# evroon/mav-detection

Hardware: AMD Instinct MI355X
Metric: frame-pairs/sec at 1920x1080 (higher is better)
Workload: dtype f32; 1 GPU; 1920x1080, batch 64 per GPU, Farneback + FoE + phi/threshold + box; global_batch=64, parallelism=frame-parallel x1, record_exchange=none (1 GPU), torch_in_process=False

## Files before the change

mav-detection_amd/csrc/kernels_flow.hip:

```cpp
#include "mavflow_internal.h"

#include <algorithm>
#include <type_traits>

static __device__ __forceinline__ int clampi(int v, int lo, int hi) { return v < lo ? lo : (v > hi ? hi : v); }

struct TileMap { int tiles_x, tiles_y, per_img, n_tiles, strip_w, xcd, ty0; };
static __device__ __forceinline__ bool tile_of_block(const TileMap& tm, int* s, int* tx, int* ty)
{
    const int per = ((int)gridDim.x + 7) >> 3;
    const int tile = tm.xcd ? (int)(blockIdx.x & 7) * per + (int)(blockIdx.x >> 3) : (int)blockIdx.x;
    if (tile >= tm.n_tiles) return false;
    const int img = tile / tm.per_img;
    int tr = tile - img * tm.per_img;
    const int strip_tiles = tm.strip_w * tm.tiles_y;
    const int st = tr / strip_tiles;
    tr -= st * strip_tiles;
    const int x_base = st * tm.strip_w;
    const int sw = min(tm.strip_w, tm.tiles_x - x_base);
    const int row = tr / sw;
    *s = img; *ty = row + tm.ty0; *tx = x_base + tr - row * sw;
    return true;
}
static TileMap make_tile_map(int w, int h, int G, int tile_w, int tile_h, int ty0 = 0, int ty1 = -1, int strip = 0)
// ... 625 lines not shown
    return p;
}
bool blur_resize_is_fused(int W, int H, int w, int h, int ksize, int esize)
{
    if (!(!(w == W && h == H) && ksize <= 13 && H > 2 * ksize && W > 2 * ksize && (size_t)fused_blur_rows(H, h, ksize) * 256 <= 48 * 1024))
        return false;
    if (esize == 1) return true;
    const int pitch = staged_pitch_words(W, w, ksize);
    return fused_lds_bytes(fused_blur_rows(H, h, ksize), pitch, esize) <= 64 * 1024;
}

template <typename T>
static __device__ __forceinline__ void blur3_block(const T* __restrict__ src, float* __restrict__ dst, int W, int H, int bx, int by)
{
    typedef typename QuadOf<T>::type Q;
    const int x = (bx * 64 + (threadIdx.x & 63)) * 4;
    const int y0 = (by * 4 + (threadIdx.x >> 6)) * 4;
    if (x >= W || y0 >= H) return;
    const int xl = x == 0 ? 1 : x - 1;
    const int xr = x + 4 >= W ? W - 2 : x + 4;
    Q qs[6];
    T ls[6], rs[6];
#pragma unroll
    for (int r = 0; r < 6; r++) {
        int yy = y0 - 1 + r;
        yy = yy < 0 ? -yy : (yy >= H ? 2 * H - 2 - yy : yy);
        yy = yy < 0 ? 0 : (yy >= H ? H - 1 : yy);
        const T* p = src + (size_t)yy * W;
        qs[r] = *(const Q*)(p + x);
        ls[r] = p[xl];
        rs[r] = p[xr];
    }
    float hrow[6][4];
#pragma unroll
    for (int r = 0; r < 6; r++) {
        if constexpr (sizeof(T) == 1) {
            const uint32_t q = qs[r];
            const float a = (float)ls[r], b0 = (float)(q & 255u), b1 = (float)((q >> 8) & 255u), b2 = (float)((q >> 16) & 255u),
                        b3 = (float)(q >> 24), c = (float)rs[r];
            hrow[r][0] = 0.5f * b0 + 0.25f * (a + b1);
            hrow[r][1] = 0.5f * b1 + 0.25f * (b0 + b2);
            hrow[r][2] = 0.5f * b2 + 0.25f * (b1 + b3);
            hrow[r][3] = 0.5f * b3 + 0.25f * (b2 + c);
        } else {
            float b[4];
            quad_px<T>(qs[r], b);
            const float a = (float)ls[r], c = (float)rs[r];
            hrow[r][0] = 0.5f * b[0] + 0.25f * (a + b[1]);
            hrow[r][1] = 0.5f * b[1] + 0.25f * (b[0] + b[2]);
            hrow[r][2] = 0.5f * b[2] + 0.25f * (b[1] + b[3]);
            hrow[r][3] = 0.5f * b[3] + 0.25f * (b[2] + c);
        }
    }
#pragma unroll
    for (int r = 0; r < 4; r++) {
        float4 o;
        o.x = 0.5f * hrow[r + 1][0] + 0.25f * (hrow[r][0] + hrow[r + 2][0]);
        o.y = 0.5f * hrow[r + 1][1] + 0.25f * (hrow[r][1] + hrow[r + 2][1]);
        o.z = 0.5f * hrow[r + 1][2] + 0.25f * (hrow[r][2] + hrow[r + 2][2]);
        o.w = 0.5f * hrow[r + 1][3] + 0.25f * (hrow[r][3] + hrow[r + 2][3]);
        if (y0 + r < H) *(float4*)(dst + (size_t)(y0 + r) * W + x) = o;
    }
}

template <typename T, int PATH>
__global__ __launch_bounds__(256) void k_blur_multi(const T* __restrict__ img, const T* __restrict__ img2, int split, size_t img_stride,
                                                    int W, int H, int dword_ok, BlurJobs jobs)
{
    extern __shared__ __attribute__((aligned(16))) float hrows[];
    int k = 0;
    for (int i = 1; i < jobs.n; i++) k = (int)blockIdx.x >= jobs.j[i].first_block ? i : k;
    const BlurJob J = jobs.j[k];
    const int b = (int)blockIdx.x - J.first_block;
    const int z = b / (J.gx * J.gy), rem = b - z * J.gx * J.gy;
    const int by = rem / J.gx, bx = rem - by * J.gx;
    const T* base = image_of(img, img2, split, img_stride, z);
    float* out = J.out + (size_t)z * J.out_stride;
    if (J.fused) blur_fused_any<T, PATH>(base, out, W, H, J.w, J.h, J.bp, J.rows_cap, J.pitch_w, dword_ok, J.th, bx, by, hrows);
    else blur3_block(base, out, W, H, bx, by);
}
template <typename T>
static int quad_ok(const FrameRun<T>& f)
{
    const uintptr_t m = 4 * sizeof(T) - 1;
    return (f.W % 4 == 0 && f.img_stride % 4 == 0 && ((uintptr_t)f.img & m) == 0 && ((uintptr_t)f.img2 & m) == 0) ? 1 : 0;
}
template <typename T>
static bool blur3_fast_ok(const FrameRun<T>& f, const LayerTarget& t)
{
    return t.w == f.W && t.h == f.H && t.bp.fixed3 && f.W >= 8 && f.H >= 2 && quad_ok(f) && t.out_stride % 4 == 0 &&
           ((uintptr_t)t.out & 15) == 0;
}
template <typename T>
bool blur_multi_ok(const FrameRun<T>& f, const LayerTarget& t)
{
    return blur3_fast_ok(f.runs(), t) || blur_resize_is_fused(f.W, f.H, t.w, t.h, t.bp.ksize, (int)sizeof(T));
}
template <typename T>
static void blur_multi_launch(hipStream_t st, const FrameRun<T>& f, int dword_ok, BlurJobs jobs)
{
    const int esize = (int)sizeof(T), W = f.W, H = f.H;
    int blocks = 0;
    size_t lds = 0;
    for (int i = 0; i < jobs.n; i++) {
        BlurJob& J = jobs.j[i];
        J.fused = !(J.w == W && J.h == H);
        if (J.fused) {
            const FusedPlan fp = fused_plan(W, H, J.w, J.h, J.bp, dword_ok, esize);
            J.rows_cap = fp.rows; J.pitch_w = fp.pitch_w; J.th = fp.th;
            J.gx = (J.w + 63) / 64; J.gy = (J.h + fp.th - 1) / fp.th;
            lds = std::max(lds, fp.lds);
        } else {
            J.rows_cap = J.pitch_w = 0;
            J.gx = (W / 4 + 63) / 64; J.gy = ((H + 3) / 4 + 3) / 4;
        }
        J.first_block = blocks;
        blocks += J.gx * J.gy * f.G;
    }
    int path = -1;
    for (int i = 0; i < jobs.n; i++)
        if (jobs.j[i].fused) {
            const int p = fused_path_of(jobs.j[i].bp, jobs.j[i].pitch_w, dword_ok, esize);
            path = path < 0 ? p : (path == p ? p : FP_ANY);
        }
    with_fused_path<T>(path, [&](auto P) {
        hipLaunchKernelGGL((k_blur_multi<T, decltype(P)::value>), dim3(blocks), dim3(256), lds, st, f.img, f.img2, f.split, f.img_stride, W, H,
                           dword_ok, jobs);
    });
}
template <typename T>
void launch_blur_multi(hipStream_t st, const FrameRun<T>& frames, BlurJobs jobs)
{
    const FrameRun<T> f = frames.runs();
    const int dword_ok = quad_ok(f);
    const int esize = (int)sizeof(T);
    if (f.G <= 8) return blur_multi_launch(st, f, dword_ok, jobs);
    bool done[MAV_MAX_JOBS] = {false};
    for (int i = 0; i < jobs.n; i++) {
        if (done[i]) continue;
        auto path_of = [&](const BlurJob& J) {
            if (J.w == f.W && J.h == f.H) return -1;
            const FusedPlan fp = fused_plan(f.W, f.H, J.w, J.h, J.bp, dword_ok, esize);
            return fused_path_of(J.bp, fp.pitch_w, dword_ok, esize);
        };
        const int p = path_of(jobs.j[i]);
        BlurJobs sub{0, 0, {}};
        for (int k = i; k < jobs.n; k++)
            if (!done[k] && path_of(jobs.j[k]) == p) { sub.j[sub.n++] = jobs.j[k]; done[k] = true; }
        blur_multi_launch(st, f, dword_ok, sub);
    }
}

template <typename T>
__global__ __launch_bounds__(256) void k_blur3(const T* __restrict__ img, const T* __restrict__ img2, int split,
                                               size_t img_stride, int W, int H, float* __restrict__ out, size_t out_stride)
{
    blur3_block(image_of(img, img2, split, img_stride, blockIdx.z), out + (size_t)blockIdx.z * out_stride, W, H, blockIdx.x, blockIdx.y);
}

template <typename T>
bool blur_resize_needs_tmp(const FrameRun<T>& f, const LayerTarget& t)
{
    return !blur3_fast_ok(f.runs(), t) && !blur_resize_is_fused(f.W, f.H, t.w, t.h, t.bp.ksize, (int)sizeof(T));
}
template <typename T>
void launch_blur_resize(hipStream_t st, const FrameRun<T>& frames, const LayerTarget& t, const BlurScratch& scratch)
{
    const FrameRun<T> f = frames.runs();
    const int G = f.G, W = f.W, H = f.H, w = t.w, h = t.h;
    const BlurParams& bp = t.bp;
    if (blur3_fast_ok(f, t)) {
        dim3 grid((W / 4 + 63) / 64, ((H + 3) / 4 + 3) / 4, G);
        hipLaunchKernelGGL(k_blur3<T>, grid, dim3(256), 0, st, f.img, f.img2, f.split, f.img_stride, W, H, t.out, t.out_stride);
        return;
    }
    const int dword_ok = quad_ok(f);
    const int esize = (int)sizeof(T);
    const int pitch_w = staged_pitch_words(W, w, bp.ksize);
    if (!scratch.two_pass && blur_resize_is_fused(W, H, w, h, bp.ksize, esize)) {
        const FusedPlan fp = fused_plan(W, H, w, h, bp, dword_ok, esize);
        const dim3 grid((w + 63) / 64, (h + fp.th - 1) / fp.th, G);
        with_fused_path<T>(fused_path_of(bp, fp.pitch_w, dword_ok, esize), [&](auto P) {
            if constexpr (decltype(P)::value != FP_ANY)
                hipLaunchKernelGGL((k_blur_resize_fused<T, decltype(P)::value>), grid, dim3(256), fp.lds, st, f.img, f.img2, f.split, f.img_stride,
                                   W, H, w, h, bp, t.out, t.out_stride, fp.rows, fp.pitch_w, dword_ok, fp.th);
        });
        return;
    }
    int rows_blk = 16;
    while (rows_blk > 4 && (size_t)rows_blk * pitch_w * 4 * esize > 48 * 1024) rows_blk >>= 1;
    if ((size_t)rows_blk * pitch_w * 4 * esize <= 48 * 1024)
    {
        const int gx = (w + 63) / 64, nby = (H + rows_blk - 1) / rows_blk;
        const int gy = nby;
        const size_t lds_h = (size_t)((rows_blk * pitch_w * esize + 1) & ~1) * 4 + (size_t)((bp.ksize + 4) & ~3) * 8;
        hipLaunchKernelGGL(k_blur_resize_h<T>, dim3(gx, gy, G), dim3(256), lds_h, st, f.img, f.img2, f.split, f.img_stride, W, H, w, bp,
                           scratch.tmp, scratch.stride, rows_blk, pitch_w, dword_ok);
    }
    else
        hipLaunchKernelGGL(k_blur_resize_h_direct<T>, dim3((w + 63) / 64, ((H + 3) / 4 + 3) / 4, G), dim3(256), 0, st, f.img, f.img2, f.split,
                           f.img_stride, W, H, w, bp, scratch.tmp, scratch.stride);
    hipLaunchKernelGGL(k_blur_resize_v, dim3((w + 63) / 64, (h + 3) / 4, G), dim3(256), 0, st, (const float*)scratch.tmp, scratch.stride, H, w,
                       h, bp, t.out, t.out_stride);
}
#define MAV_BLUR_DEPTH(T)                                                                                     \
    template bool blur_multi_ok<T>(const FrameRun<T>&, const LayerTarget&);                                   \
    template void launch_blur_multi<T>(hipStream_t, const FrameRun<T>&, BlurJobs);                            \
    template bool blur_resize_needs_tmp<T>(const FrameRun<T>&, const LayerTarget&);                           \
    template void launch_blur_resize<T>(hipStream_t, const FrameRun<T>&, const LayerTarget&, const BlurScratch&);
MAV_BLUR_DEPTH(uint8_t)
MAV_BLUR_DEPTH(uint16_t)
MAV_BLUR_DEPTH(float)
#undef MAV_BLUR_DEPTH

#define PX 64
#define PY 16
struct __attribute__((packed, aligned(4))) F2U { float x, y; };
struct __attribute__((packed, aligned(4))) F4U { float x, y, z, w; };
static __device__ __forceinline__ void load5(const float* __restrict__ p, float v[5])
{
    const F4U a = *(const F4U*)p;
    v[0] = a.x; v[1] = a.y; v[2] = a.z; v[3] = a.w; v[4] = p[4];
}
static __device__ __forceinline__ void store5(float* __restrict__ p, const float v[5])
{
    *(F4U*)p = F4U{v[0], v[1], v[2], v[3]};
    p[4] = v[4];
}
template <int N_T>
static __device__ __forceinline__ void polyexp_tile(const float* __restrict__ src, float* __restrict__ dst, int w, int h, const PolyCoef& pc,
                                                    int tile_x, int tile_y, float* __restrict__ smem)
{
    const int n = N_T > 0 ? N_T : pc.n;
    const int EX = PX + 2 * n, EY = PY + 2 * n;
    float* tile = smem;
    float* v0 = tile + EX * EY;
    float* v1 = v0 + PY * EX;
    float* v2 = v1 + PY * EX;
    const int tid = threadIdx.x;
    const int x0 = tile_x * PX, y0 = tile_y * PY;

    if constexpr (N_T > 0) {
        constexpr int TOT = (PX + 2 * N_T) * (PY + 2 * N_T), CNT = (TOT + 255) / 256;
        float v[CNT];
#pragma unroll
        for (int j = 0; j < CNT; j++) {
            const int i = tid + 256 * j;
            if (i < TOT) {
                const int ly = i / EX, lx = i - ly * EX;
                const int gx = clampi(x0 - n + lx, 0, w - 1), gy = clampi(y0 - n + ly, 0, h - 1);
                v[j] = src[(size_t)gy * w + gx];
            }
        }
#pragma unroll
        for (int j = 0; j < CNT; j++)
            if (tid + 256 * j < TOT) tile[tid + 256 * j] = v[j];
    } else {
        for (int i = tid; i < EX * EY; i += 256) {
            const int ly = i / EX, lx = i - ly * EX;
            const int gx = clampi(x0 - n + lx, 0, w - 1), gy = clampi(y0 - n + ly, 0, h - 1);
            tile[i] = src[(size_t)gy * w + gx];
        }
    }
    __syncthreads();
    for (int i = tid; i < PY * EX; i += 256) {
        const int ly = i / EX, lx = i - ly * EX;
        const float* c = tile + (ly + n) * EX + lx;
        float t0 = c[0] * pc.g[0], t1 = 0.f, t2 = 0.f;
#pragma unroll
        for (int k = 1; k <= n; k++) {
            const float a = c[-k * EX], b = c[k * EX];
            const float p = a + b;
            t0 = fmaf(pc.g[k], p, t0);
            t1 = fmaf(pc.xg[k], b - a, t1);
            t2 = fmaf(pc.xxg[k], p, t2);
        }
        v0[i] = t0; v1[i] = t1; v2[i] = t2;
    }
    __syncthreads();
    for (int i = tid; i < PY * PX; i += 256) {
        const int ly = i >> 6, lx = i & 63;
        const int gx = x0 + lx, gy = y0 + ly;
        if (gx >= w || gy >= h) continue;
        const float* p0 = v0 + ly * EX + lx + n;
        const float* p1 = v1 + ly * EX + lx + n;
        const float* p2 = v2 + ly * EX + lx + n;
        float b1 = p0[0] * pc.g[0], b2 = 0.f, b3 = p1[0] * pc.g[0], b4 = 0.f, b5 = p2[0] * pc.g[0], b6 = 0.f;
#pragma unroll
        for (int k = 1; k <= n; k++) {
            const float a0 = p0[-k], c0 = p0[k], a1 = p1[-k], c1 = p1[k], a2 = p2[-k], c2 = p2[k];
            const float tg = c0 + a0;
            b1 = fmaf(tg, pc.g[k], b1);
            b4 = fmaf(tg, pc.xxg[k], b4);
            b2 = fmaf(c0 - a0, pc.xg[k], b2);
            b3 = fmaf(c1 + a1, pc.g[k], b3);
            b6 = fmaf(c1 - a1, pc.xg[k], b6);
            b5 = fmaf(c2 + a2, pc.g[k], b5);
        }
        const float r[5] = {b3 * pc.ig11, b2 * pc.ig11, fmaf(b5, pc.ig33, b1 * pc.ig03), fmaf(b4, pc.ig33, b1 * pc.ig03), b6 * pc.ig55};
        store5(dst + 5 * ((size_t)gy * w + gx), r);
    }
}

template <int N_T>
__global__ __launch_bounds__(256) void k_polyexp(const float* __restrict__ I, size_t I_stride, int w, int h, PolyCoef pc, TileMap tm,
                                                 float* __restrict__ R, size_t R_stride)
{
    int img_s, tile_x, tile_y;
    if (!tile_of_block(tm, &img_s, &tile_x, &tile_y)) return;
    extern __shared__ __attribute__((aligned(16))) float smem[];
    polyexp_tile<N_T>(I + (size_t)img_s * I_stride, R + (size_t)img_s * R_stride, w, h, pc, tile_x, tile_y, smem);
}

template <int N_T>
__global__ __launch_bounds__(256) void k_polyexp_multi(PolyJobs jobs, PolyCoef pc)
{
    int k = 0;
    for (int i = 1; i < jobs.n; i++) k = (int)blockIdx.x >= jobs.j[i].first_block ? i : k;
    const PolyJob J = jobs.j[k];
    const int tile = (int)blockIdx.x - J.first_block;
    const int img_s = tile / J.per_img, rem = tile - img_s * J.per_img;
    const int tile_y = rem / J.tiles_x, tile_x = rem - tile_y * J.tiles_x;
    extern __shared__ __attribute__((aligned(16))) float smem[];
    polyexp_tile<N_T>(J.I + (size_t)img_s * J.I_stride, J.R + (size_t)img_s * J.R_stride, J.w, J.h, pc, tile_x, tile_y, smem);
}
void launch_polyexp_multi(hipStream_t st, PolyJobs jobs, int G, const PolyCoef& pc)
{
    const int n = pc.n;
    const size_t lds = sizeof(float) * ((size_t)(PX + 2 * n) * (PY + 2 * n) + 3 * (size_t)PY * (PX + 2 * n));
    int blocks = 0;
    for (int i = 0; i < jobs.n; i++) {
        PolyJob& J = jobs.j[i];
        J.tiles_x = (J.w + PX - 1) / PX;
        J.per_img = J.tiles_x * ((J.h + PY - 1) / PY);
        J.first_block = blocks;
        blocks += J.per_img * G;
    }
    if (n == 8) hipLaunchKernelGGL(k_polyexp_multi<8>, dim3(blocks), dim3(256), lds, st, jobs, pc);
    else if (n == 7) hipLaunchKernelGGL(k_polyexp_multi<7>, dim3(blocks), dim3(256), lds, st, jobs, pc);
    else if (n == 5) hipLaunchKernelGGL(k_polyexp_multi<5>, dim3(blocks), dim3(256), lds, st, jobs, pc);
    else hipLaunchKernelGGL(k_polyexp_multi<0>, dim3(blocks), dim3(256), lds, st, jobs, pc);
}

void launch_polyexp(hipStream_t st, const float* I, size_t I_stride, int G, int w, int h, const PolyCoef& pc, float* R,
                    size_t R_stride)
{
    const int n = pc.n;
    const size_t lds = sizeof(float) * ((size_t)(PX + 2 * n) * (PY + 2 * n) + 3 * (size_t)PY * (PX + 2 * n));
    TileMap tm = make_tile_map(w, h, G, PX, PY);
    tm.xcd = 0;
    const dim3 grid(tile_grid(tm));
    if (n == 8)
        hipLaunchKernelGGL(k_polyexp<8>, grid, dim3(256), lds, st, I, I_stride, w, h, pc, tm, R, R_stride);
    else if (n == 7)
        hipLaunchKernelGGL(k_polyexp<7>, grid, dim3(256), lds, st, I, I_stride, w, h, pc, tm, R, R_stride);
    else if (n == 5)
        hipLaunchKernelGGL(k_polyexp<5>, grid, dim3(256), lds, st, I, I_stride, w, h, pc, tm, R, R_stride);
    else
        hipLaunchKernelGGL(k_polyexp<0>, grid, dim3(256), lds, st, I, I_stride, w, h, pc, tm, R, R_stride);
}

struct GatherPx {
    float p00[5], p01[5], p10[5], p11[5];
    float fx, fy;
    bool inside;
};
static __device__ __forceinline__ void gather_row(const float* __restrict__ p, float a[5], float b[5])
{
    const F4U t0 = *(const F4U*)p, t1 = *(const F4U*)(p + 4);
    const F2U t2 = *(const F2U*)(p + 8);
    a[0] = t0.x; a[1] = t0.y; a[2] = t0.z; a[3] = t0.w; a[4] = t1.x;
    b[0] = t1.y; b[1] = t1.z; b[2] = t1.w; b[3] = t2.x; b[4] = t2.y;
}
static __device__ __forceinline__ void gather_issue(const float* __restrict__ R1p, int w, int h, int x, int y, float dx, float dy, GatherPx& g)
{
    float fx = x + dx, fy = y + dy;
    const int x1 = (int)floorf(fx), y1 = (int)floorf(fy);
    g.fx = fx - x1; g.fy = fy - y1;
    g.inside = (unsigned)x1 < (unsigned)(w - 1) && (unsigned)y1 < (unsigned)(h - 1);
    const int xc = g.inside ? x1 : 0, yc = g.inside ? y1 : 0;
    const float* p = R1p + 5 * ((size_t)yc * w + xc);
    const size_t row = (w > 1 && h > 1) ? 5 * (size_t)w : 0;
    gather_row(p, g.p00, g.p01);
    gather_row(p + row, g.p10, g.p11);
}
static __device__ __forceinline__ void gather_inside(const float* __restrict__ R1p, int w, int h, int x, int y, float dx, float dy, GatherPx& g)
{
    float fx = x + dx, fy = y + dy;
    const int x1 = (int)floorf(fx), y1 = (int)floorf(fy);
    g.fx = fx - x1; g.fy = fy - y1;
    g.inside = (unsigned)x1 < (unsigned)(w - 1) && (unsigned)y1 < (unsigned)(h - 1);
    if (!g.inside) return;
    const float* p = R1p + 5 * ((size_t)y1 * w + x1);
    gather_row(p, g.p00, g.p01);
    gather_row(p + 5 * (size_t)w, g.p10, g.p11);
}
static __device__ __forceinline__ void update_finish(const float q[5], const GatherPx& g, int w, int h, int x, int y, float dx,
                                                     float dy, float out[5])
{
#pragma clang fp contract(off)
    float r2, r3, r4, r5, r6;
    if (g.inside) {
        const float gx = 1.f - g.fx, gy = 1.f - g.fy;
        const float a00 = gx * gy, a01 = g.fx * gy, a10 = gx * g.fy, a11 = g.fx * g.fy;
        r2 = fmaf(a11, g.p11[0], fmaf(a10, g.p10[0], fmaf(a01, g.p01[0], a00 * g.p00[0])));
        r3 = fmaf(a11, g.p11[1], fmaf(a10, g.p10[1], fmaf(a01, g.p01[1], a00 * g.p00[1])));
        r4 = fmaf(a11, g.p11[2], fmaf(a10, g.p10[2], fmaf(a01, g.p01[2], a00 * g.p00[2])));
        r5 = fmaf(a11, g.p11[3], fmaf(a10, g.p10[3], fmaf(a01, g.p01[3], a00 * g.p00[3])));
        r6 = fmaf(a11, g.p11[4], fmaf(a10, g.p10[4], fmaf(a01, g.p01[4], a00 * g.p00[4])));
        r4 = (q[2] + r4) * 0.5f;
        r5 = (q[3] + r5) * 0.5f;
        r6 = (q[4] + r6) * 0.25f;
    } else {
        r2 = r3 = 0.f;
        r4 = q[2]; r5 = q[3]; r6 = q[4] * 0.5f;
    }
    r2 = (q[0] - r2) * 0.5f;
    r3 = (q[1] - r3) * 0.5f;
    r2 += fmaf(r4, dy, r6 * dx);
    r3 += fmaf(r6, dy, r5 * dx);
    const int BORDER = 5;
    if ((unsigned)(x - BORDER) >= (unsigned)(w - BORDER * 2) || (unsigned)(y - BORDER) >= (unsigned)(h - BORDER * 2)) {
        auto bw = [](int d) { return d < 2 ? 0.14f : 0.4472f; };
        const float scale = (x < BORDER ? bw(x) : 1.f) * (x >= w - BORDER ? bw(w - x - 1) : 1.f) *
                            (y < BORDER ? bw(y) : 1.f) * (y >= h - BORDER ? bw(h - y - 1) : 1.f);
        r2 *= scale; r3 *= scale; r4 *= scale; r5 *= scale; r6 *= scale;
    }
    out[0] = fmaf(r4, r4, r6 * r6);
    out[1] = (r4 + r5) * r6;
    out[2] = fmaf(r5, r5, r6 * r6);
    out[3] = fmaf(r4, r2, r6 * r3);
    out[4] = fmaf(r6, r2, r5 * r3);
}

static __device__ __forceinline__ void update_px(const float* __restrict__ R0p, const float* __restrict__ R1p, size_t npx,
                                                 int w, int h, int x, int y, float dx, float dy, float* __restrict__ Mp)
{
    const size_t idx = (size_t)y * w + x;
    float q[5], o[5];
    load5(R0p + 5 * idx, q);
    GatherPx g;
    gather_inside(R1p, w, h, x, y, dx, dy, g);
    update_finish(q, g, w, h, x, y, dx, dy, o);
#pragma unroll
    for (int c = 0; c < 5; c++) Mp[c * npx + idx] = o[c];
}

static __device__ __forceinline__ void solve_px(float g11, float g12, float g22, float h1, float h2, float* u, float* v)
{
    const float p = g12 * g12, pe = fmaf(g12, g12, -p);
    const float det = (fmaf(g11, g22, -p) - pe) + 1e-3f;
    const float idet = 1.f / det;
    const float qa = g12 * h1, qae = fmaf(g12, h1, -qa);
    const float qb = g12 * h2, qbe = fmaf(g12, h2, -qb);
    *u = (fmaf(g11, h2, -qa) - qae) * idet;
    *v = (fmaf(g22, h1, -qb) - qbe) * idet;
}

static __device__ __forceinline__ float2 upsample_flow(const float* __restrict__ pf, int pw, int ph, float mul, double scale_x,
                                                       double scale_y, int x, int y)
{
#pragma clang fp contract(off)
    float fy = (float)((y + 0.5) * scale_y - 0.5);
    int sy = (int)floorf(fy);
    fy -= sy;
    if (sy < 0) { fy = 0.f; sy = 0; }
    if (sy >= ph - 1) { fy = 0.f; sy = ph - 1; }
    const int sy1 = sy + 1 < ph ? sy + 1 : sy;
    float fx = (float)((x + 0.5) * scale_x - 0.5);
    int sx = (int)floorf(fx);
    fx -= sx;
    if (sx < 0) { fx = 0.f; sx = 0; }
    if (sx >= pw - 1) { fx = 0.f; sx = pw - 1; }
    const int sx1 = sx + 1 < pw ? sx + 1 : sx;
    const float a0 = 1.f - fx, a1 = fx, b0 = 1.f - fy, b1 = fy;
    const float2 p00 = *(const float2*)(pf + ((size_t)sy * pw + sx) * 2);
    const float2 p01 = *(const float2*)(pf + ((size_t)sy * pw + sx1) * 2);
    const float2 p10 = *(const float2*)(pf + ((size_t)sy1 * pw + sx) * 2);
    const float2 p11 = *(const float2*)(pf + ((size_t)sy1 * pw + sx1) * 2);
    return make_float2(((p00.x * a0 + p01.x * a1) * b0 + (p10.x * a0 + p11.x * a1) * b1) * mul,
                       ((p00.y * a0 + p01.y * a1) * b0 + (p10.y * a0 + p11.y * a1) * b1) * mul);
}

template <int MODE>
__global__ __launch_bounds__(256) void k_update_matrices(const float* __restrict__ R0, const float* __restrict__ R1,
                                                         size_t R_stride, const float* __restrict__ fsrc, size_t f_stride,
                                                         int pw, int ph, float mul, double scale_x, double scale_y, int w,
                                                         int h, float* __restrict__ M, size_t M_stride, int y_begin, int y_end)
{
    const int x = blockIdx.x * 64 + (threadIdx.x & 63);
    const int y = y_begin + blockIdx.y * 4 + (threadIdx.x >> 6);
    if (x >= w || y >= y_end) return;
    const int s = blockIdx.z;
    float dx = 0.f, dy = 0.f;
    if (MODE == 1) {
        const float2 f = upsample_flow(fsrc + (size_t)s * f_stride, pw, ph, mul, scale_x, scale_y, x, y);
        dx = f.x; dy = f.y;
    } else if (MODE == 2) {
        const float2 f = *(const float2*)(fsrc + (size_t)s * f_stride + ((size_t)y * w + x) * 2);
        dx = f.x; dy = f.y;
    }
    update_px(R0 + (size_t)s * R_stride, R1 + (size_t)s * R_stride, (size_t)w * h, w, h, x, y, dx, dy,
              M + (size_t)s * M_stride);
}

void launch_initial_m(hipStream_t st, const InitialMArgs& a, const FlowSource& src)
{
    const int y_begin = a.y_begin < 0 ? 0 : a.y_begin, y_end = (a.y_end < 0 || a.y_end > a.h) ? a.h : a.y_end;
    if (y_end <= y_begin) return;
    const auto k = src.kind == FlowSource::COARSER ? k_update_matrices<1> : src.kind == FlowSource::FIELD ? k_update_matrices<2> : k_update_matrices<0>;
    hipLaunchKernelGGL(k, dim3((a.w + 63) / 64, (y_end - y_begin + 3) / 4, a.G), dim3(256), 0, st, a.R0, a.R1, a.R_stride, src.flow, src.stride,
                       src.pw, src.ph, src.mul, (double)src.pw / a.w, (double)src.ph / a.h, a.w, a.h, a.M, a.M_stride, y_begin, y_end);
}

struct BoxWindow {
    float scale;
    template <int M_T, int N, bool REGS, typename In, typename Out>
    __device__ __forceinline__ void sums(int m_rt, In in, Out out) const
    {
        const int win = 2 * (M_T > 0 ? M_T : m_rt) + 1;
        constexpr int UNROLL = REGS ? N : 8;
        decltype(in(0)) sum{};
#pragma unroll
        for (int k = 0; k < win; k++) sum += in(k);
#pragma unroll UNROLL
        for (int j = 0; j < N; j++) {
            const auto s = sum;
            if (j < N - 1) sum += in(j + win) - in(j);
            out(j, s);
        }
    }
    __device__ __forceinline__ void solve(float g11, float g12, float g22, float h1, float h2, float* u, float* v) const
    {
        solve_px(g11 * scale, g12 * scale, g22 * scale, h1 * scale, h2 * scale, u, v);
    }
};

void gauss_taps(int winsize, GaussTaps* out)
{
    const int m = winsize / 2;
    const double sigma = m * 0.3;
    float t[MAV_MAX_WIN_HALF + 1];
    double s = 1.;
    for (int i = 0; i <= m; i++) {
        t[i] = (float)exp(-i * i / (2 * sigma * sigma));
        s += t[i] * 2;
    }
    s = 1. / s;
    for (int i = 0; i <= MAV_MAX_WIN_HALF; i++) out->k[i] = i <= m ? (float)(t[i] * s) : 0.f;
}

static __device__ __forceinline__ void solve_gauss_px(float g11, float g12, float g22, float h1, float h2, float* u, float* v)
{
#pragma clang fp contract(off)
    const float d = g11 * g22 - g12 * g12;
    const double idet = 1.0 / ((double)d + 1e-3);
    *u = (float)((double)(g11 * h2 - g12 * h1) * idet);
    *v = (float)((double)(g22 * h1 - g12 * h2) * idet);
}

struct GaussWindow {
    GaussTaps gt;
    template <int M_T, int N, bool REGS, typename In, typename Out>
    __device__ __forceinline__ void sums(int m_rt, In in, Out out) const
    {
#pragma clang fp contract(off)
        const int m = M_T > 0 ? M_T : m_rt;
        constexpr int UNROLL = REGS ? N : 2;
#pragma unroll UNROLL
        for (int j = 0; j < N; j++) {
            auto a = in(j + m) * gt.k[0];
            if (M_T > 0) {
#pragma unroll
                for (int i = 1; i <= M_T; i++) a += (in(j + m - i) + in(j + m + i)) * gt.k[i];
            } else {
                for (int i = 1; i <= m; i++) a += (in(j + m - i) + in(j + m + i)) * gt.k[i];
            }
            out(j, a);
        }
    }
    __device__ __forceinline__ void solve(float g11, float g12, float g22, float h1, float h2, float* u, float* v) const
    {
        solve_gauss_px(g11, g12, g22, h1, h2, u, v);
    }
};

static inline void iter_geometry(int m, int* ext, int* pitch, int* plane)
{
    *ext = MAV_TILE + 2 * m;
    *pitch = (*ext & 1) ? *ext : *ext + 1;
    int p = *ext * *pitch;
    while ((p - *ext) % 32 != 0) p++;
    *plane = p;
}

size_t blur_iter_lds_bytes(int winsize)
{
    int ext, pitch, plane;
    iter_geometry(winsize / 2, &ext, &pitch, &plane);
    return sizeof(float) * 5 * (size_t)plane;
}

template <typename Win, int M_T>
__global__ __launch_bounds__(256) void k_blur_iter_generic(const float* __restrict__ M_in, float* __restrict__ M_out, size_t M_stride,
                                                   const float* __restrict__ R0, const float* __restrict__ R1, size_t R_stride,
                                                   int w, int h, int m_rt, int pitch, int plane, Win win, int do_update,
                                                   float* __restrict__ flow, size_t f_stride)
{
    extern __shared__ __attribute__((aligned(16))) float lds[];
    const int m = M_T > 0 ? M_T : m_rt;
    const int ext = MAV_TILE + 2 * m;
    const int tid = threadIdx.x;
    const int s = blockIdx.z;
    const int x0 = blockIdx.x * MAV_TILE, y0 = blockIdx.y * MAV_TILE;
    const size_t npx = (size_t)w * h;
    const float* Min = M_in + (size_t)s * M_stride;

    for (int c = 0; c < 5; c++) {
        const float* P = Min + c * npx;
        float* L = lds + c * plane;
        for (int i = tid; i < ext * ext; i += 256) {
            const int ly = i / ext, lx = i - ly * ext;
            const int gx = clampi(x0 - m + lx, 0, w - 1), gy = clampi(y0 - m + ly, 0, h - 1);
            L[ly * pitch + lx] = P[(size_t)gy * w + gx];
        }
    }
    __syncthreads();
    for (int t = tid; t < 5 * ext; t += 256) {
        const int c = t / ext, lx = t - c * ext;
        float* col = lds + c * plane + lx;
        win.template sums<M_T, MAV_TILE, false>(m, [&](int i) { return col[i * pitch]; }, [&](int y, float a) { col[y * pitch] = a; });
    }
    __syncthreads();
    for (int t = tid; t < 5 * MAV_TILE; t += 256) {
        const int c = t >> 5, y = t & 31;
        float* row = lds + c * plane + y * pitch;
        win.template sums<M_T, MAV_TILE, false>(m, [&](int i) { return row[i]; }, [&](int x, float a) { row[x] = a; });
    }
    __syncthreads();
    const float* R0p = R0 + (size_t)s * R_stride;
    const float* R1p = R1 + (size_t)s * R_stride;
    float* Mo = M_out + (size_t)s * M_stride;
    float* fo = flow + (size_t)s * f_stride;
    const int lx = tid & 31;
    const int gx = x0 + lx;
#pragma unroll
    for (int j = 0; j < 4; j++) {
        const int ly = (tid >> 5) + 8 * j;
        const int gy = y0 + ly;
        if (gx >= w || gy >= h) continue;
        const float* L = lds + ly * pitch + lx;
        float u, v;
        win.solve(L[0], L[plane], L[2 * plane], L[3 * plane], L[4 * plane], &u, &v);
        *(float2*)(fo + ((size_t)gy * w + gx) * 2) = make_float2(u, v);
        if (do_update) update_px(R0p, R1p, npx, w, h, gx, gy, u, v, Mo);
    }
}

#define FT_X 64
#define FT_Y 16

template <typename Win, int M_T, bool AL, bool WT>
// ... 209 lines not shown
```

mav-detection_amd/csrc/mavflow_internal.h:

```cpp
#pragma once
#include <hip/hip_runtime.h>
#include <stdint.h>
#include <vector>

#include "../../include/mavflow.h"

#define MAV_MAX_POLY_N 16
#define MAV_TILE 32

struct PolyCoef {
    int n;
    float g[MAV_MAX_POLY_N + 1], xg[MAV_MAX_POLY_N + 1], xxg[MAV_MAX_POLY_N + 1];
    float ig11, ig03, ig33, ig55;
};

struct BlurParams {
    int ksize;
    int fixed3;
    const float* g;
    double scale_x;
    double scale_y;
    const int* xs; const float* xf;
    const int* ys; const float* yf;
};

enum { MAV_PAIR_PROMOTE = 0, MAV_PAIR_DEROTATE = 1, MAV_PAIR_FRAME0 = 2 };
struct DerotParams {
    double o0, o1, o2, sx, sy;
    int mode;
};

static __device__ __forceinline__ void derot_apply(float2 f, const DerotParams* __restrict__ dp, int W, int H, int row, int col,
                                                   double* fu, double* fv)
{
    double u = (double)f.x, v = (double)f.y;
    if (dp && dp->mode == MAV_PAIR_DEROTATE) {
        const double x = -((double)col / (double)W - 0.5) * 2.0;
        const double y = -((double)row / (double)H - 0.5) * 2.0;
        const double o0 = dp->o0, o1 = dp->o1, o2 = dp->o2;
        double du = (((o0 * x) * y - o1 * (x * x)) - o1) + o2 * y;
        double dv = ((((-o2) * x + o0) + o0 * (y * y))) - (o1 * x) * y;
        du = du * dp->sx;
        dv = dv * dp->sy;
        u = u - du;
        v = v - dv;
    }
    *fu = u; *fv = v;
}
static __device__ __forceinline__ void derot_apply(double2 f, const DerotParams*, int, int, int, int, double* fu, double* fv)
{
    *fu = f.x; *fv = f.y;
}

#define MAV_MAX_JOBS 6
struct PolyJob { const float* I; float* R; size_t I_stride, R_stride; int w, h, tiles_x, per_img, first_block, pad; };
struct PolyJobs { int n, pad; PolyJob j[MAV_MAX_JOBS]; };

template <typename T>
struct FrameRun {
    const T *img, *img2;
    int split;
    size_t img_stride;
    int G, W, H;
    FrameRun runs() const { return img2 ? *this : FrameRun{img, img, G, img_stride, G, W, H}; }
};
struct LayerTarget { float* out; size_t out_stride; BlurParams bp; int w, h; };
struct BlurJob : LayerTarget { int fused, gx, gy, first_block, rows_cap, pitch_w, th, pad; };
struct BlurJobs { int n, pad; BlurJob j[MAV_MAX_JOBS]; };
struct BlurScratch { float* tmp; size_t stride; bool two_pass = false; };
template <typename T>
void launch_blur_resize(hipStream_t st, const FrameRun<T>& f, const LayerTarget& t, const BlurScratch& scratch);
bool blur_resize_is_fused(int W, int H, int w, int h, int ksize, int esize = 1);
template <typename T>
bool blur_resize_needs_tmp(const FrameRun<T>& f, const LayerTarget& t);
void launch_polyexp(hipStream_t st, const float* I, size_t I_stride, int G, int w, int h, const PolyCoef& pc, float* R,
                    size_t R_stride);
void launch_polyexp_multi(hipStream_t st, PolyJobs jobs, int G, const PolyCoef& pc);
template <typename T>
bool blur_multi_ok(const FrameRun<T>& f, const LayerTarget& t);
template <typename T>
void launch_blur_multi(hipStream_t st, const FrameRun<T>& f, BlurJobs jobs);

struct PairOperands { const float *R0, *R1; size_t R_stride; int G, w, h; };
inline std::vector<float> expansion_of_planes(const float* planes, size_t n)
{
    std::vector<float> e(planes ? 5 * n : 0);
    for (size_t c = 0; c < 5 && planes; c++)
        for (size_t i = 0; i < n; i++) e[5 * i + c] = planes[c * n + i];
    return e;
}
inline int planes_of_expansion(int rc, const std::vector<float>& e, size_t n, float* planes)
{
    for (size_t c = 0; c < 5 && rc == MAV_OK; c++)
        for (size_t i = 0; i < n; i++) planes[c * n + i] = e[5 * i + c];
    return rc;
}
struct FlowSource {
    enum Kind { ZERO = 0, COARSER = 1, FIELD = 2 };
    Kind kind = ZERO;
    const float* flow = nullptr;
    size_t stride = 0;
    int pw = 0, ph = 0;
    float mul = 0.f;
    static FlowSource coarser(const float* flow, size_t stride, int pw, int ph, float mul)
    {
        return flow ? FlowSource{COARSER, flow, stride, pw, ph, mul} : FlowSource{};
    }
    static FlowSource field(const float* flow, size_t stride) { return FlowSource{FIELD, flow, stride}; }
    FlowSource from_pair(int s0) const { FlowSource u = *this; if (u.flow) u.flow += (size_t)s0 * stride; return u; }
};
struct InitialMArgs : PairOperands {
    float* M;
    size_t M_stride;
    int y_begin = 0, y_end = -1;
};
void launch_initial_m(hipStream_t st, const InitialMArgs& a, const FlowSource& src);
#define MAV_MAX_WIN_HALF 32
struct GaussTaps { float k[MAV_MAX_WIN_HALF + 1]; };
void gauss_taps(int winsize, GaussTaps* out);
struct SweepArgs : PairOperands {
    const float* M_in;
    float* M_out;
    size_t M_stride;
    int winsize;
    float* flow;
    size_t f_stride;
    int do_update, store_flow;
    int ty0 = 0, ty1 = -1;
    int strip = 0;
    bool write_through = false;
    const GaussTaps* gauss = nullptr;
};
void launch_blur_iter(hipStream_t st, const SweepArgs& a);
int blur_iter_tile_rows(int h);
bool blur_iter_bands_ok(const SweepArgs& a);
size_t blur_iter_lds_bytes(int winsize);
const char* blur_iter_prepare(int winsize);

void launch_probe_r3w1(hipStream_t st, const float* a, const float* b, const float* c, float* d, size_t n_float4);

struct FoeScratch {
    double* cand;
    int* count;
    unsigned long long* best_key;
    unsigned* done;
};
void launch_foe_f32(hipStream_t st, const float* flow, const DerotParams* derot , const uint32_t* samples,
                    int B, int W, int H, int N, double mag2_thr, float mag2_thr_f32 , double dist2_thr,
                    FoeScratch s, double* foe, int32_t* box_acc ,
                    unsigned long long* max_phi_bits );
void launch_foe_f64(hipStream_t st, const double* flow, const uint32_t* samples, int B, int W, int H, int N, double mag2_thr,
                    double dist2_thr, FoeScratch s, double* foe, int32_t* box_acc, unsigned long long* max_phi_bits);
void launch_box_init(hipStream_t st, int32_t* box_acc, unsigned long long* max_phi_bits, unsigned* done , int B);
struct PhiLaunch {
    unsigned* done = nullptr;
    mav_result* results = nullptr;
    int32_t* box_out = nullptr;
    bool screen = true;
    int yloop = 0;
};
void launch_phi_mask_f32(hipStream_t st, const float* flow, const DerotParams* derot, const double* foe, const uint8_t* sky,
                         int B, int W, int H, mav_thr_params thr, double* phi, uint8_t* mask_fixed, uint8_t* mask_dyn,
                         int32_t* box_acc, unsigned long long* max_phi_bits, const PhiLaunch& pl);
void launch_phi_mask_f64(hipStream_t st, const double* flow, const double* foe, const uint8_t* sky, int B, int W, int H,
                         mav_thr_params thr, double* phi, uint8_t* mask_fixed, uint8_t* mask_dyn, int32_t* box_acc,
                         unsigned long long* max_phi_bits, const PhiLaunch& pl);
void launch_box_finalize(hipStream_t st, const int32_t* box_acc, int B, int32_t* box);
void launch_derotate(hipStream_t st, const float* flow, const DerotParams* derot, int B, int W, int H, double* out);
void launch_bbox_u8(hipStream_t st, const uint8_t* img, int B, int W, int H, int* maxv , int32_t* box_acc);
void launch_window_max(hipStream_t st, const uint8_t* img, int B, int W, int H, unsigned long long* key ,
                       int64_t* out);
void launch_tpr_fpr(hipStream_t st, const uint8_t* gt, const uint8_t* mask, unsigned mask_value, int B, int W, int H,
                    unsigned long long* counts );
void launch_tpr_fpr2(hipStream_t st, const uint8_t* gt, size_t gt_stride, const uint8_t* mask0, const uint8_t* mask1, unsigned mask_value, int B,
                     int W, int H, unsigned long long* counts0 , unsigned long long* counts1 );
struct RocThr {
    int ka, km;
    double mag0_sq_lo;
    double ang[MAV_ROC_MAX_ANGLES], mag[MAV_ROC_MAX_MAGS];
    float ang32[MAV_ROC_MAX_ANGLES], mag32[MAV_ROC_MAX_MAGS];
};
hipError_t launch_roc_sweep(hipStream_t st, const void* flow, bool f64, const DerotParams* derot , const double* foe,
                      const uint8_t* sky, const uint8_t* gt, size_t gt_stride, int B, int W, int H, const RocThr& thr, unsigned long long* table);
void launch_bgr2gray(hipStream_t st, const uint8_t* bgr, size_t n, uint8_t* gray);
void launch_ransac_only(hipStream_t st, FoeScratch s, int M, int N, double dist2_thr, double* foe);
void launch_make_derot(hipStream_t st, const double* omega , const double* dt, const uint8_t* frame0, int B,
                       int W, int H, DerotParams* out);
void launch_render_f32(hipStream_t st, const float* flow, const DerotParams* derot, const double* foe, const uint8_t* sky, int B, int W,
                       int H, mav_thr_params thr, unsigned long long* radmax, uint8_t* res, uint8_t* flow_img, uint8_t* phi_img);
void launch_render_f64(hipStream_t st, const double* flow, int B, int W, int H, unsigned long long* radmax, uint8_t* flow_img);
void launch_colormap_jet(hipStream_t st, const uint8_t* gray, size_t n, uint8_t* bgr);
void launch_overlay(hipStream_t st, const uint8_t* frames, const uint8_t* mask, const double* foe, const double* foe_gt, int B, int W, int H,
                    int radius, uint8_t* out, uint8_t* written);

#define MAV_PYR_MAX 32
struct PyrPlan {
    int n;
    int w[MAV_PYR_MAX], h[MAV_PYR_MAX];
    unsigned base[MAV_PYR_MAX + 1];
    size_t off[MAV_PYR_MAX];
};
void launch_area_resize(hipStream_t st, const uint8_t* src, size_t src_stride, int sw, int sh, uint8_t* dst, size_t dst_stride,
                        int dw, int dh, int B);
void launch_area_resize_flow(hipStream_t st, const float* src, size_t src_stride, int sw, int sh, float* dst, size_t dst_stride, int dw,
                             int dh, int B, double scale);
void launch_level_scan(hipStream_t st, const uint8_t* img, size_t stride, int B, int W, int H, unsigned idx_base,
                       unsigned long long* key );
void launch_pyramid_finalize(hipStream_t st, const unsigned long long* key, const PyrPlan& plan, const uint8_t* img0,
                             const uint8_t* ws, int B, int64_t* out );
void launch_optimize_window(hipStream_t st, const uint8_t* img, int B, int W, int H, unsigned long long* sat ,
                            const int32_t* win_in, int64_t* score, int32_t* win_out);

#define MAV_PNG_SEG 24576
#define MAV_PNG_SLOT (MAV_PNG_SEG + 16)
size_t png_segments(size_t raw);
size_t png_workspace_per_image(size_t raw);
void launch_png_encode(hipStream_t st, const uint8_t* imgs, int img0, int nimg, int W, int H, int C, uint8_t* ws, uint8_t* out,
                       unsigned long long* index);

#define MAV_LK_MAX_LEVELS 8
#define MAV_LK_HIST 104
struct LkLevels { int n; int w[MAV_LK_MAX_LEVELS], h[MAV_LK_MAX_LEVELS]; unsigned off[MAV_LK_MAX_LEVELS]; };
struct LkTrackArgs {
    const uint8_t *I, *J;
    const short2* D;
    LkLevels lv;
    const float* pts;
    int n, win_w, win_h, max_count;
    double eps2;
    float min_eig;
    float* out;
    uint8_t* status;
    unsigned* iter_hist;
    const int* n_dev;
};
struct LkTrackErrArgs : LkTrackArgs {
    float* err;
    int flags;
};
struct LkPickArgs {
    const uint2* cand;
    const unsigned* n_ptr;
    unsigned cap;
    int W, max_corners;
    int pick;
    int cell, gw, gh, slots;
    double md2;
    unsigned* grid;
    float* corners;
    int* count;
    unsigned* stats;
};
void launch_min_eig(hipStream_t st, const uint8_t* img, const uint8_t* mask, int W, int H, int block_size, float s2, float* eig, unsigned* maxkey);
void launch_harris(hipStream_t st, const uint8_t* img, const uint8_t* mask, int W, int H, int block_size, float s2, float k, float* eig,
                   unsigned* maxkey);
void launch_corner_candidates(hipStream_t st, const float* eig, const uint8_t* mask, int W, int H, const unsigned* maxkey, double quality,
                              uint2* cand, unsigned* count, unsigned cap);
void launch_pick_sort(hipStream_t st, uint2* cand, const unsigned* n_ptr, unsigned cap);
void launch_corner_pick(hipStream_t st, const LkPickArgs& a);
void launch_lk_pyrdown(hipStream_t st, const uint8_t* src, int sw, int sh, uint8_t* dst, int dw, int dh);
void launch_lk_scharr(hipStream_t st, const uint8_t* pyr, const LkLevels& lv, int levels, short2* out);
size_t lk_track_lds_bytes(int win_w, int win_h);
void launch_lk_track(hipStream_t st, const LkTrackArgs& a);
void launch_lk_track_err(hipStream_t st, const LkTrackErrArgs& a);

void launch_pair_gather(hipStream_t st, const float* flow, const int32_t* coords, int n, int B, int W, int H, double* src, double* dst);
size_t homography_work_doubles(int n);
void launch_homography_fit(hipStream_t st, const double* src, const double* dst, int n, int B, double* work, double* H, int* ok);
void launch_motion_pass_a(hipStream_t st, const float* flow, const double* M, int m_stride, int B, int W, int H, float* warped, float* mag,
                          float* gm, unsigned long long* key);
void launch_motion_pass_b(hipStream_t st, const float* flow, const double* M, int m_stride, int B, int W, int H, const unsigned long long* key,
                          uint8_t* gray);
void launch_motion_window(hipStream_t st, const int64_t* pyr, int B, int32_t* win);
void launch_motion_pack(hipStream_t st, const unsigned long long* key, const int64_t* pyr, const int32_t* win, const int64_t* opt_score,
                        const int32_t* opt_win, const int* ok, int B, int W, mav_motion_result* out);

struct CcArgs {
    const uint8_t* mask;
    int B, W, H, connectivity, min_area, max_blobs;
    void* ws;
    int32_t* labels;
    mav_cc_counts* counts;
    mav_blob* blobs;
};
size_t cc_workspace_per_image(int W, int H);
void launch_components(hipStream_t st, const CcArgs& a);

struct HistSlots { int n; unsigned w[(MAV_HISTORY_MAX_LENGTH + 3) / 4]; };
void launch_remap_linear(hipStream_t st, const void* src, bool f64, const float* map_x, const float* map_y, int W, int H, double* out);
void launch_history_put(hipStream_t st, const void* src, bool src_f64, void* slot, bool ring_f64, int W, int H);
void launch_history_trace(hipStream_t st, const void* ring, bool ring_f64, const HistSlots& slots, int W, int H, bool axes_xy, bool out_f32, void* out);

#define MAV_GT_FLOW_GRID_CAP 1024u
void launch_gt_flow(hipStream_t st, const float* depth, const uint8_t* seg, const void* params , int B, int W, int H,
                    bool out_f64, void* out);
struct RadialEdges { int n, pad; double e[257]; };
#define MAV_RADIAL_LDS_CELLS 32768
#define MAV_RADIAL_GRID_CAP 256
bool radial_hist_lds_counts(int nm, int ne);
int radial_hist_grid(size_t npx, int B);
hipError_t launch_radial_hist(hipStream_t st, const float* flow, const float* gt, const uint8_t* sky, int B, int W, int H, const RadialEdges& mag,
                              const RadialEdges& err, double* edges_dev, bool edges_resident, unsigned long long* table);

#define MAV_GT_STATS_GRID_CAP 2048u
struct GtsAcc { unsigned long long drone, pos, tp, fp; int seg_max; unsigned depth_key, nan; int pad; int box[4]; };
static_assert(sizeof(GtsAcc) == 64, "GtsAcc");
inline size_t gts_rows_offset(int B) { return sizeof(GtsAcc) * (size_t)B; }
inline size_t gts_list_offset(int B, int H) { return gts_rows_offset(B) + ((sizeof(int) * (size_t)B * H + 15) & ~(size_t)15); }
size_t gt_stats_scratch_bytes(int B, int H, int max_pixels, bool own_list);
struct GtStatsCall {
    const uint8_t *seg, *sky; const float *gt_flow, *depth; const void* params; int B, W, H, max_pixels; void* scratch; void* records; int32_t* indices;
};
enum { GTS_PHASE_MAX, GTS_PHASE_COUNT, GTS_PHASE_LIST, GTS_PHASE_SUM, GTS_PHASES };
void launch_gt_stats_phase(hipStream_t st, int phase, const GtStatsCall& k);

#define KM_THREADS 256
#define KM_PER_THREAD 16
#define KM_GRID_CAP 1024u
struct KmState {
    double S[16][16][4];
    double shift[16], compact[16];
    unsigned long long key[16];
    float c[16][16][4];
    float mean[16][4];
    int n[16][16];
    int done[16], iters[16], repairs[16], pending[16], donor[16];
    int live, any_pending, best, skipped;
};
struct KmCall {
    const void* samples; const float* init; int32_t* labels; float* centers; void* records; char* ws;
    int n, B, A, K, D, u8, max_iter; double eps2;
};
inline size_t km_chunks(int n) { return ((size_t)n + KM_THREADS * KM_PER_THREAD - 1) / (KM_THREADS * KM_PER_THREAD); }
inline size_t km_state_bytes() { return (sizeof(KmState) + 255) & ~(size_t)255; }
inline size_t km_labels_bytes(int n, int A) { return ((size_t)A * n + 255) & ~(size_t)255; }
inline size_t km_slab_bytes(int n, int A, int K, int D) { return sizeof(double) * km_chunks(n) * A * K * (D + 1); }
inline size_t km_image_bytes(int n, int A, int K, int D) { return km_state_bytes() + km_labels_bytes(n, A) + ((km_slab_bytes(n, A, K, D) + 255) & ~(size_t)255); }
void launch_kmeans(hipStream_t st, const KmCall& k);
void launch_kmeans_paint(hipStream_t st, const int32_t* labels, const float* centers, int n, int B, int K, int D, uint8_t* res, uint8_t* mask);

enum { WARP_POLICY_MAP, WARP_POLICY_PLANES, WARP_POLICY_FLOW, WARP_POLICY_AFFINE, WARP_POLICY_PERSPECTIVE };
void launch_warp(hipStream_t st, int policy, int format, const void* src, const void* a, const void* b, int flags, int W, int H, int B, void* dst);
void launch_warp_method(hipStream_t st, int policy, const float* flow, const double* M, int W, int H, int B, float* diff, float* mag, void* records);

struct AffCall {
    const double *src, *dst; const int32_t* triples; double* M; uint8_t* inliers; void* records; char* ws;
    int n, B, max_iters, refine; double t2;
};
__host__ __device__ inline size_t aff_round(size_t bytes) { return (bytes + 255) & ~(size_t)255; }
__host__ __device__ inline size_t aff_counts_offset(int n) { return aff_round(sizeof(int32_t) * ((size_t)n + 1)); }
__host__ __device__ inline size_t aff_choice_offset(int n, int B, int max_iters) { return aff_counts_offset(n) + aff_round(sizeof(int32_t) * (size_t)B * max_iters); }
__host__ __device__ inline size_t aff_coords_offset(int n, int B, int max_iters) { return aff_choice_offset(n, B, max_iters) + aff_round(sizeof(int32_t) * 4 * (size_t)B); }
__host__ __device__ inline size_t aff_src_offset(int n, int B, int max_iters) { return aff_coords_offset(n, B, max_iters) + aff_round(sizeof(int32_t) * 2 * (size_t)n); }
__host__ __device__ inline size_t aff_dst_offset(int n, int B, int max_iters) { return aff_src_offset(n, B, max_iters) + aff_round(sizeof(double) * 2 * (size_t)n * B); }
__host__ __device__ inline size_t aff_workspace_bytes(int n, int B, int max_iters) { return aff_dst_offset(n, B, max_iters) + aff_round(sizeof(double) * 2 * (size_t)n * B); }
void launch_affine_score(hipStream_t st, const AffCall& a);
void launch_affine_choose(hipStream_t st, const AffCall& a);
void launch_affine_finish(hipStream_t st, const AffCall& a);
// ... 19 lines not shown
```

Before: 2842 frame-pairs/s.

## Add vectorized polynomial-expansion tile path with float4 loads and packed FMA

Adds a fast polyexp tile path for widths divisible by 4 with aligned buffers. It loads the halo tile with float4 global reads, runs the vertical and horizontal separable passes with packed 2-wide FMAs over padded LDS rows, and transposes the 5-channel results through LDS so the global stores are coalesced float4 writes. The aim is to cut memory instruction count and ALU issue in the Farneback polynomial-expansion stage. It uses more LDS, which may lower occupancy, and the slower path is kept for misaligned cases.

After: 2906 frame-pairs/s (median of 6 runs). 1.02x the previous value.

```diff
diff --git a/mav-detection_amd/csrc/kernels_flow.hip b/mav-detection_amd/csrc/kernels_flow.hip
--- a/mav-detection_amd/csrc/kernels_flow.hip
+++ b/mav-detection_amd/csrc/kernels_flow.hip
@@ -951,14 +951,175 @@
     }
 }
 
+typedef float pk2 __attribute__((ext_vector_type(2)));
+#define PF_QX 20
+#define PF_TP 84
+#define PF_PP 80
+static __device__ __forceinline__ pk2 pk_fma(float s, pk2 x, pk2 acc) { return __builtin_elementwise_fma(pk2{s, s}, x, acc); }
+template <int N_T>
+static __device__ __forceinline__ void load_quads5(const float* __restrict__ p, float f[20])
+{
+    typedef float pk4 __attribute__((ext_vector_type(4)));
+    pk4 t[5];
+#pragma unroll
+    for (int k = 0; k < 5; k++) t[k] = ((const pk4*)p)[k];
+#pragma unroll
+    for (int k = 0; k < 5; k++) {
+        if constexpr (N_T < 8) asm volatile("" : "+v"(t[k]));
+        f[4 * k] = t[k].x; f[4 * k + 1] = t[k].y; f[4 * k + 2] = t[k].z; f[4 * k + 3] = t[k].w;
+    }
+}
+template <int N_T>
+static __device__ __forceinline__ void polyexp_tile_fast(const float* __restrict__ src, float* __restrict__ dst, int w, int h, const PolyCoef& pc,
+                                                         int tile_x, int tile_y, float* __restrict__ smem)
+{
+    constexpr int n = N_T, EY = PY + 2 * n, NV = 4 + 2 * n;
+    float* tile = smem;
+    float* v0 = tile + EY * PF_TP;
+    float* v1 = v0 + PY * PF_PP;
+    float* v2 = v1 + PY * PF_PP;
+    const int tid = threadIdx.x;
+    const int x0 = tile_x * PX, y0 = tile_y * PY;
+    {
+        constexpr int TOT = PF_QX * EY, CNT = (TOT + 255) / 256;
+        float4 q[CNT];
+#pragma unroll
+        for (int j = 0; j < CNT; j++) {
+            const int i = min(tid + 256 * j, TOT - 1);
+            const int ly = i / PF_QX, qx = i - ly * PF_QX;
+            const int gx = x0 - 8 + 4 * qx, gy = clampi(y0 - n + ly, 0, h - 1);
+            q[j] = *(const float4*)(src + (size_t)gy * w + clampi(gx, 0, w - 4));
+        }
+#pragma unroll
+        for (int j = 0; j < CNT; j++) {
+            const int i = tid + 256 * j;
+            const int ly = i / PF_QX, qx = i - ly * PF_QX;
+            const int gx = x0 - 8 + 4 * qx;
+            const bool lo = gx < 0, hi = gx >= w, out = lo || hi;
+            const float4 t = q[j];
+            const float e = lo ? t.x : t.w;
+            if (i < TOT) *(float4*)(tile + ly * PF_TP + 4 * qx) = make_float4(hi ? e : t.x, out ? e : t.y, out ? e : t.z, lo ? e : t.w);
+        }
+    }
+    __syncthreads();
+    if (tid < (PY / 4) * (PF_PP / 2)) {
+        const int rb = tid / (PF_PP / 2), cp = tid - rb * (PF_PP / 2);
+        const float* c = tile + rb * 4 * PF_TP + 2 * cp;
+        pk2 v[NV];
+#pragma unroll
+        for (int i = 0; i < NV; i++) v[i] = *(const pk2*)(c + i * PF_TP);
+#pragma unroll
+        for (int j = 0; j < 4; j++) {
+            pk2 t0 = v[j + n] * pc.g[0], t1 = pk2{0.f, 0.f}, t2 = pk2{0.f, 0.f};
+#pragma unroll
+            for (int k = 1; k <= n; k++) {
+                const pk2 a = v[j + n - k], b = v[j + n + k];
+                const pk2 p = a + b;
+                t0 = pk_fma(pc.g[k], p, t0);
+                t1 = pk_fma(pc.xg[k], b - a, t1);
+                t2 = pk_fma(pc.xxg[k], p, t2);
+            }
+            const int o = (rb * 4 + j) * PF_PP + 2 * cp;
+            *(pk2*)(v0 + o) = t0; *(pk2*)(v1 + o) = t1; *(pk2*)(v2 + o) = t2;
+        }
+    }
+    __syncthreads();
+    {
+        const int lane = tid & 63, wv = tid >> 6;
+        const int quad = (lane & 31) >> 2;
+        const int grp = (lane >> 5) * 2 + ((quad == 1 || quad == 2 || quad == 4 || quad == 7) ? 1 : 0);
+        const int qpos = (quad == 0 || quad == 1) ? 0 : ((quad == 3 || quad == 2) ? 1 : ((quad == 5 || quad == 4) ? 2 : 3));
+        const int ly = wv * 4 + grp, lx0 = (qpos * 4 + (lane & 3)) * 4;
+        const int gy = y0 + ly;
+        const int o = ly * PF_PP + lx0;
+        float f[20];
+        pk2 b1[2], b2[2], b3[2], b4[2], b5[2], b6[2];
+        load_quads5<N_T>(v0 + o, f);
+#pragma unroll
+        for (int j = 0; j < 2; j++) {
+            const int m = 8 + 2 * j;
+            b1[j] = pk2{f[m], f[m + 1]} * pc.g[0]; b2[j] = pk2{0.f, 0.f}; b4[j] = pk2{0.f, 0.f};
+#pragma unroll
+            for (int k = 1; k <= n; k++) {
+                const pk2 a0 = pk2{f[m - k], f[m + 1 - k]}, c0 = pk2{f[m + k], f[m + 1 + k]};
+                const pk2 tg = c0 + a0;
+                b1[j] = pk_fma(pc.g[k], tg, b1[j]);
+                b4[j] = pk_fma(pc.xxg[k], tg, b4[j]);
+                b2[j] = pk_fma(pc.xg[k], c0 - a0, b2[j]);
+            }
+        }
+        load_quads5<N_T>(v1 + o, f);
+#pragma unroll
+        for (int j = 0; j < 2; j++) {
+            const int m = 8 + 2 * j;
+            b3[j] = pk2{f[m], f[m + 1]} * pc.g[0]; b6[j] = pk2{0.f, 0.f};
+#pragma unroll
+            for (int k = 1; k <= n; k++) {
+                const pk2 a1 = pk2{f[m - k], f[m + 1 - k]}, c1 = pk2{f[m + k], f[m + 1 + k]};
+                b3[j] = pk_fma(pc.g[k], c1 + a1, b3[j]);
+                b6[j] = pk_fma(pc.xg[k], c1 - a1, b6[j]);
+            }
+        }
+        load_quads5<N_T>(v2 + o, f);
+#pragma unroll
+        for (int j = 0; j < 2; j++) {
+            const int m = 8 + 2 * j;
+            b5[j] = pk2{f[m], f[m + 1]} * pc.g[0];
+#pragma unroll
+            for (int k = 1; k <= n; k++) {
+                const pk2 a2 = pk2{f[m - k], f[m + 1 - k]}, c2 = pk2{f[m + k], f[m + 1 + k]};
+                b5[j] = pk_fma(pc.g[k], c2 + a2, b5[j]);
+            }
+        }
+        float r[20];
+#pragma unroll
+        for (int j = 0; j < 2; j++) {
+            const pk2 r0 = b3[j] * pc.ig11, r1 = b2[j] * pc.ig11, e = b1[j] * pc.ig03;
+            const pk2 r2 = pk_fma(pc.ig33, b5[j], e), r3 = pk_fma(pc.ig33, b4[j], e), r4 = b6[j] * pc.ig55;
+            float* q = r + 10 * j;
+            q[0] = r0.x; q[1] = r1.x; q[2] = r2.x; q[3] = r3.x; q[4] = r4.x;
+            q[5] = r0.y; q[6] = r1.y; q[7] = r2.y; q[8] = r3.y; q[9] = r4.y;
+        }
+        {
+            const int pos = lx0 >> 2;
+            auto chunk = [&](int c) { return smem + (c < 3 ? EY * PF_TP + c * PY * PF_PP : 0) + ly * PF_PP; };
+            float* wr = chunk(pos >> 2) + 4 * (5 * (pos & 3));
+#pragma unroll
+            for (int k = 0; k < 5; k++) *(float4*)(wr + 4 * k) = make_float4(r[4 * k], r[4 * k + 1], r[4 * k + 2], r[4 * k + 3]);
+            const int vq = 5 * (min(PX, w - x0) >> 2);
+            float4* out = (float4*)(dst + 5 * ((size_t)gy * w + x0));
+            float4 t[5];
+#pragma unroll
+            for (int k = 0; k < 5; k++) {
+                const int idx = 16 * k + pos, c = idx / 20;
+                t[k] = *(const float4*)(chunk(c) + 4 * (idx - 20 * c));
+            }
+            if (gy < h) {
+#pragma unroll
+                for (int k = 0; k < 5; k++)
+                    if (16 * k + pos < vq) out[16 * k + pos] = t[k];
+            }
+        }
+    }
+}
+template <int N_T>
+static __device__ __forceinline__ void polyexp_tile_any(bool fast, const float* __restrict__ src, float* __restrict__ dst, int w, int h,
+                                                        const PolyCoef& pc, int tile_x, int tile_y, float* __restrict__ smem)
+{
+    if constexpr (N_T > 0) {
+        if (fast) { polyexp_tile_fast<N_T>(src, dst, w, h, pc, tile_x, tile_y, smem); return; }
+    }
+    polyexp_tile<N_T>(src, dst, w, h, pc, tile_x, tile_y, smem);
+}
+
 template <int N_T>
 __global__ __launch_bounds__(256) void k_polyexp(const float* __restrict__ I, size_t I_stride, int w, int h, PolyCoef pc, TileMap tm,
-                                                 float* __restrict__ R, size_t R_stride)
+                                                 float* __restrict__ R, size_t R_stride, int fast)
 {
     int img_s, tile_x, tile_y;
     if (!tile_of_block(tm, &img_s, &tile_x, &tile_y)) return;
     extern __shared__ __attribute__((aligned(16))) float smem[];
-    polyexp_tile<N_T>(I + (size_t)img_s * I_stride, R + (size_t)img_s * R_stride, w, h, pc, tile_x, tile_y, smem);
+    polyexp_tile_any<N_T>(fast != 0, I + (size_t)img_s * I_stride, R + (size_t)img_s * R_stride, w, h, pc, tile_x, tile_y, smem);
 }
 
 template <int N_T>
@@ -971,20 +1132,34 @@
     const int img_s = tile / J.per_img, rem = tile - img_s * J.per_img;
     const int tile_y = rem / J.tiles_x, tile_x = rem - tile_y * J.tiles_x;
     extern __shared__ __attribute__((aligned(16))) float smem[];
-    polyexp_tile<N_T>(J.I + (size_t)img_s * J.I_stride, J.R + (size_t)img_s * J.R_stride, J.w, J.h, pc, tile_x, tile_y, smem);
+    polyexp_tile_any<N_T>(J.fast != 0, J.I + (size_t)img_s * J.I_stride, J.R + (size_t)img_s * J.R_stride, J.w, J.h, pc, tile_x, tile_y, smem);
+}
+static bool polyexp_vec_ok(const float* I, size_t I_stride, const float* R, size_t R_stride, int w, int n)
+{
+    return (n == 8 || n == 7 || n == 5) && w >= 4 && w % 4 == 0 && I_stride % 4 == 0 && R_stride % 4 == 0 && ((uintptr_t)I & 15) == 0 &&
+           ((uintptr_t)R & 15) == 0;
+}
+static size_t polyexp_lds_bytes(int n, bool fast)
+{
+    const size_t relaxed = sizeof(float) * ((size_t)(PX + 2 * n) * (PY + 2 * n) + 3 * (size_t)PY * (PX + 2 * n));
+    const size_t vec = sizeof(float) * ((size_t)(PY + 2 * n) * PF_TP + 3 * (size_t)PY * PF_PP);
+    return fast && vec > relaxed ? vec : relaxed;
 }
 void launch_polyexp_multi(hipStream_t st, PolyJobs jobs, int G, const PolyCoef& pc)
 {
     const int n = pc.n;
-    const size_t lds = sizeof(float) * ((size_t)(PX + 2 * n) * (PY + 2 * n) + 3 * (size_t)PY * (PX + 2 * n));
     int blocks = 0;
+    bool any_fast = false;
     for (int i = 0; i < jobs.n; i++) {
         PolyJob& J = jobs.j[i];
         J.tiles_x = (J.w + PX - 1) / PX;
         J.per_img = J.tiles_x * ((J.h + PY - 1) / PY);
         J.first_block = blocks;
+        J.fast = polyexp_vec_ok(J.I, J.I_stride, J.R, J.R_stride, J.w, n);
+        any_fast |= J.fast != 0;
         blocks += J.per_img * G;
     }
+    const size_t lds = polyexp_lds_bytes(n, any_fast);
     if (n == 8) hipLaunchKernelGGL(k_polyexp_multi<8>, dim3(blocks), dim3(256), lds, st, jobs, pc);
     else if (n == 7) hipLaunchKernelGGL(k_polyexp_multi<7>, dim3(blocks), dim3(256), lds, st, jobs, pc);
     else if (n == 5) hipLaunchKernelGGL(k_polyexp_multi<5>, dim3(blocks), dim3(256), lds, st, jobs, pc);
@@ -995,18 +1170,19 @@
                     size_t R_stride)
 {
     const int n = pc.n;
-    const size_t lds = sizeof(float) * ((size_t)(PX + 2 * n) * (PY + 2 * n) + 3 * (size_t)PY * (PX + 2 * n));
+    const int fast = polyexp_vec_ok(I, I_stride, R, R_stride, w, n);
+    const size_t lds = polyexp_lds_bytes(n, fast != 0);
     TileMap tm = make_tile_map(w, h, G, PX, PY);
     tm.xcd = 0;
     const dim3 grid(tile_grid(tm));
     if (n == 8)
-        hipLaunchKernelGGL(k_polyexp<8>, grid, dim3(256), lds, st, I, I_stride, w, h, pc, tm, R, R_stride);
+        hipLaunchKernelGGL(k_polyexp<8>, grid, dim3(256), lds, st, I, I_stride, w, h, pc, tm, R, R_stride, fast);
     else if (n == 7)
-        hipLaunchKernelGGL(k_polyexp<7>, grid, dim3(256), lds, st, I, I_stride, w, h, pc, tm, R, R_stride);
+        hipLaunchKernelGGL(k_polyexp<7>, grid, dim3(256), lds, st, I, I_stride, w, h, pc, tm, R, R_stride, fast);
     else if (n == 5)
-        hipLaunchKernelGGL(k_polyexp<5>, grid, dim3(256), lds, st, I, I_stride, w, h, pc, tm, R, R_stride);
+        hipLaunchKernelGGL(k_polyexp<5>, grid, dim3(256), lds, st, I, I_stride, w, h, pc, tm, R, R_stride, fast);
     else
-        hipLaunchKernelGGL(k_polyexp<0>, grid, dim3(256), lds, st, I, I_stride, w, h, pc, tm, R, R_stride);
+        hipLaunchKernelGGL(k_polyexp<0>, grid, dim3(256), lds, st, I, I_stride, w, h, pc, tm, R, R_stride, fast);
 }
 
 struct GatherPx {
diff --git a/mav-detection_amd/csrc/mavflow_internal.h b/mav-detection_amd/csrc/mavflow_internal.h
--- a/mav-detection_amd/csrc/mavflow_internal.h
+++ b/mav-detection_amd/csrc/mavflow_internal.h
@@ -53,7 +53,7 @@
 }
 
 #define MAV_MAX_JOBS 6
-struct PolyJob { const float* I; float* R; size_t I_stride, R_stride; int w, h, tiles_x, per_img, first_block, pad; };
+struct PolyJob { const float* I; float* R; size_t I_stride, R_stride; int w, h, tiles_x, per_img, first_block, fast; };
 struct PolyJobs { int n, pad; PolyJob j[MAV_MAX_JOBS]; };
 
 template <typename T>
```
